# eromero-vlc/superbblas

Measured on AMD Instinct MI355X. Metric: lattice contraction GFLOP/s + permute GB/s, 16^4 spin×color, 1/2/4/8 GPUs, higher is better.
Workload: dtype complex<f64>

## Files before the change

superbblas_amd/csrc/capi.cpp:

```cpp
#include "plan.h"
#include <atomic>
#include <algorithm>
#include <functional>
#include <memory>
#include <unordered_map>

#include <rccl/rccl.h>

#include <cstdlib>
#include <cstring>
#include <mutex>

namespace sbx {
BsrOp *bsr_create(int nd, int ni, int dtype, const std::vector<std::vector<Range>> &pi,
                  const Coor &dimi, const std::vector<std::vector<Range>> &pd, const Coor &dimd,
                  const Coor &blocki, const Coor &blockd, bool block_im_fast,
                  const std::vector<const int *> &ii, const std::vector<const int *> &jj,
                  const std::vector<const void *> &v, const std::vector<int> &devs, bool reverse_jj,
                  const Comm &comm, const Coor *kroni = nullptr, const Coor *krond = nullptr,
                  const std::vector<const void *> *kronv = nullptr);
void bsr_destroy(BsrOp *op);
void bsr_krylov(const BsrOp &op, const Scalar &alpha, const std::string &oi,
                const std::string &od, const DistTensor &x, const Coor &fromx, const Coor &sizex,
                const Scalar &beta, const DistTensor &y, const Coor &fromy, const Coor &sizey,
// ... 301 lines not shown
        clear_copy_launch_cache();
        std::lock_guard<std::mutex> g(g_tape_mutex);
        tapes().clear();
    });
}

int sbx_clear_handles(void) {
    return guard([&] {
        trim_pools();
        destroy_streams();
    });
}

int sbx_allocate(unsigned long long bytes, sbx_context ctx, void **ptr) {
    return guard([&] {
        if (ctx.plat == SBX_GPU) {
            *ptr = device_alloc(bytes, ctx.device);
        } else {
            SBX_HIP_CHECK(hipHostMalloc(ptr, bytes, hipHostMallocDefault));
        }
    });
}

int sbx_deallocate(void *ptr, sbx_context ctx) {
    return guard([&] {
        if (!ptr) return;
        if (ctx.plat == SBX_GPU) {
            set_device(ctx.device);
            SBX_HIP_CHECK(hipStreamSynchronize(get_stream(ctx.device)));
            device_free(ptr, ctx.device);
        } else {
            SBX_HIP_CHECK(hipHostFree(ptr));
        }
    });
}

int sbx_set_custom_allocator(sbx_alloc_fn alloc, sbx_free_fn dealloc, void *user) {
    return guard([&] {
        if ((alloc == nullptr) != (dealloc == nullptr))
            throw Error("set_custom_allocator: give both functions or neither");
        set_alloc_hooks(alloc, dealloc, user);
    });
}

int sbx_allocate_from_cache(unsigned long long bytes, sbx_context ctx, void **ptr) {
    return guard([&] {
        if (ctx.plat != SBX_GPU) throw Error("allocate_from_cache: GPU contexts only");
        *ptr = scratch_alloc(bytes, ctx.device);
    });
}

int sbx_release_to_cache(void *ptr, sbx_context ctx) {
    return guard([&] {
        if (ctx.plat != SBX_GPU) throw Error("release_to_cache: GPU contexts only");
        scratch_free(ptr, ctx.device);
    });
}

int sbx_cache_usage(int device, unsigned long long *cached, unsigned long long *live) {
    return guard([&] {
        std::size_t c = 0, l = 0;
        cache_usage(device, &c, &l);
        if (cached) *cached = c;
        if (live) *live = l;
    });
}

int sbx_tune_set(const char *key, long long value) {
    return guard([&] {
        if (!key) throw Error("tune_set: null key");
        const std::string k(key);
        if (k == "copy.budget") g_copy_tune.budget = (long)value;
        else if (k == "copy.run") g_copy_tune.run = (long)value;
        else if (k == "copy.nt") g_copy_tune.nt = (int)value;
        else if (k == "copy.max_elems") g_copy_tune.max_elems = (long)value;
        else if (k == "copy.pair") g_copy_tune.pair = (int)value;
        else if (k == "copy.order") g_copy_tune.order = (int)value;
        else if (k == "copy.trans") g_copy_tune.trans = (int)value;
        else if (k == "copy.btrans") g_copy_tune.btrans = (int)value;
        else if (k == "gemm.max_bytes") g_gemm_tune.max_bytes = (long)value;
        else if (k == "gemm.loaders") g_gemm_tune.loaders = (int)value;
        else if (k == "gemm.dma_spread") g_gemm_tune.dma_spread = (int)value;
        else if (k == "gemm.dma_nt") g_gemm_tune.dma_nt = (int)value;
        else if (k == "gemm.skinny") g_gemm_tune.skinny = (int)value;
        else if (k == "bsr.variant") g_bsr_tune.variant = (int)value;
        else if (k == "bsr.row_max_cols") g_bsr_tune.row_max_cols = (long)value;
        else if (k == "bsr.split_max_cols") g_bsr_tune.split_max_cols = (long)value;
        else if (k == "bsr.split_cw") g_bsr_tune.split_cw = (int)value;
        else if (k == "bsr.split_jb") g_bsr_tune.split_jb = (int)value;
        else if (k == "bsr.split_ilv") g_bsr_tune.split_ilv = (int)value;
        else if (k == "bsr.kron_mfma") g_bsr_tune.kron_mfma = (int)value;
        else if (k == "bsr.kron_mfma_min_cols") g_bsr_tune.kron_mfma_min_cols = (long)value;
        else if (k == "bsr.kron_pack") g_bsr_tune.kron_pack = (int)value;
        else if (k == "bsr.kron_xlds") g_bsr_tune.kron_xlds = (int)value;
        else if (k == "bsr.kron_ylds") g_bsr_tune.kron_ylds = (int)value;
        else if (k == "bsr.kron_spin") g_bsr_tune.kron_spin = (int)value;
        else if (k == "bsr.kron_spin_min_cols") g_bsr_tune.kron_spin_min_cols = (long)value;
        else if (k == "bsr.kron_order") g_bsr_tune.kron_order = (int)value;
        else if (k == "bsr.nt") g_bsr_tune.nt = (int)value;
        else if (k == "dense.wave") g_dense_wave = (int)value;
        else if (k == "bsr.blk_pd") g_bsr_tune.blk_pd = (int)value;
        else if (k == "bsr.tile") g_bsr_tune.tile = (int)value;
        else if (k == "bsr.tile_min_cols") g_bsr_tune.tile_min_cols = value;
        else if (k == "gemm.m3") g_gemm_tune.m3 = (int)value;
        else if (k == "gemm.splits") g_gemm_tune.splits = (int)value;
        else if (k == "gemm.t48") g_gemm_tune.t48 = (int)value;
        else if (k == "gemm.share_ab") g_gemm_tune.share_ab = (int)value;
        else if (k == "gemm.herm") g_gemm_tune.herm = (int)value;
        else if (k == "gemm.frag") g_gemm_tune.frag = (int)value;
        else if (k == "gemm.dot_wgs") g_gemm_tune.dot_wgs = (int)value;
        else if (k == "gemm.frag_tall") g_gemm_tune.frag_tall = (int)value;
        else if (k == "gemm.frag_pair") g_gemm_tune.frag_pair = (int)value;
        else if (k == "gemm.frag_nt") g_gemm_tune.frag_nt = (int)value;
        else if (k == "gemm.frag_small") g_gemm_tune.frag_small = (int)value;
        else if (k == "gemm.frag_uk") g_gemm_tune.frag_uk = (int)value;
        else if (k == "gemm.frag_waves") g_gemm_tune.frag_waves = (int)value;
        else if (k == "gemm.clock") {
            g_gemm_tune.clock = (int)value;
            unsigned long long v[3];
            gemm_clock_read(current_device(), v, true);
        }
        else if (k == "dist.reduce") g_dist_reduce = (int)value;
        else if (k == "debug.level") g_debug_level = (int)value;
        else if (k == "debug.corrupt_copy") g_debug_corrupt = (int)value;
        else if (k == "dist.reduce_calls") g_dist_reduce_calls = value;
        else if (k == "dist.force_peer") g_dist_force_peer = (int)value;
        else if (k == "dist.peer_copies") g_dist_peer_copies = value;
        else if (k.compare(0, 6, "alloc.") == 0) alloc_tune(key, nullptr, &value);
        else throw Error("tune_set: unknown key " + k);
        if (k.compare(0, 5, "copy.") == 0) {
            std::lock_guard<std::mutex> g(g_tape_mutex);
            tapes().clear();
        }
    });
}

int sbx_tune_get(const char *key, long long *value) {
    return guard([&] {
        if (!key || !value) throw Error("tune_get: null argument");
        const std::string k(key);
        if (k == "copy.budget") *value = g_copy_tune.budget;
        else if (k == "copy.run") *value = g_copy_tune.run;
        else if (k == "copy.nt") *value = g_copy_tune.nt;
        else if (k == "copy.max_elems") *value = g_copy_tune.max_elems;
        else if (k == "copy.pair") *value = g_copy_tune.pair;
        else if (k == "copy.order") *value = g_copy_tune.order;
        else if (k == "copy.trans") *value = g_copy_tune.trans;
        else if (k == "copy.btrans") *value = g_copy_tune.btrans;
        else if (k == "copy.last_pair") *value = g_copy_tune.last_pair;
        else if (k == "gemm.max_bytes") *value = g_gemm_tune.max_bytes;
        else if (k == "gemm.loaders") *value = g_gemm_tune.loaders;
        else if (k == "gemm.dma_spread") *value = g_gemm_tune.dma_spread;
        else if (k == "gemm.dma_nt") *value = g_gemm_tune.dma_nt;
        else if (k == "gemm.skinny") *value = g_gemm_tune.skinny;
        else if (k == "bsr.variant") *value = g_bsr_tune.variant;
        else if (k == "bsr.row_max_cols") *value = g_bsr_tune.row_max_cols;
        else if (k == "bsr.split_max_cols") *value = g_bsr_tune.split_max_cols;
        else if (k == "bsr.split_cw") *value = g_bsr_tune.split_cw;
        else if (k == "bsr.split_jb") *value = g_bsr_tune.split_jb;
        else if (k == "bsr.split_ilv") *value = g_bsr_tune.split_ilv;
        else if (k == "bsr.kron_mfma") *value = g_bsr_tune.kron_mfma;
        else if (k == "bsr.kron_mfma_min_cols") *value = g_bsr_tune.kron_mfma_min_cols;
        else if (k == "bsr.kron_pack") *value = g_bsr_tune.kron_pack;
        else if (k == "bsr.kron_xlds") *value = g_bsr_tune.kron_xlds;
        else if (k == "bsr.kron_ylds") *value = g_bsr_tune.kron_ylds;
        else if (k == "bsr.kron_spin") *value = g_bsr_tune.kron_spin;
        else if (k == "bsr.kron_spin_min_cols") *value = g_bsr_tune.kron_spin_min_cols;
        else if (k == "bsr.kron_order") *value = g_bsr_tune.kron_order;
        else if (k == "bsr.nt") *value = g_bsr_tune.nt;
        else if (k == "dense.wave") *value = g_dense_wave;
        else if (k == "bsr.blk_pd") *value = g_bsr_tune.blk_pd;
        else if (k == "bsr.tile") *value = g_bsr_tune.tile;
        else if (k == "bsr.tile_min_cols") *value = g_bsr_tune.tile_min_cols;
        else if (k == "bsr.last_kernel") *value = g_bsr_tune.last;
        else if (k == "gemm.m3") *value = g_gemm_tune.m3;
        else if (k == "gemm.splits") *value = g_gemm_tune.splits;
        else if (k == "gemm.t48") *value = g_gemm_tune.t48;
        else if (k == "gemm.share_ab") *value = g_gemm_tune.share_ab;
        else if (k == "gemm.herm") *value = g_gemm_tune.herm;
        else if (k == "gemm.last_herm") *value = g_gemm_tune.last_herm;
        else if (k == "gemm.frag") *value = g_gemm_tune.frag;
        else if (k == "gemm.dot_wgs") *value = g_gemm_tune.dot_wgs;
        else if (k == "gemm.frag_tall") *value = g_gemm_tune.frag_tall;
        else if (k == "gemm.frag_pair") *value = g_gemm_tune.frag_pair;
        else if (k == "gemm.frag_nt") *value = g_gemm_tune.frag_nt;
        else if (k == "gemm.frag_small") *value = g_gemm_tune.frag_small;
        else if (k == "gemm.frag_uk") *value = g_gemm_tune.frag_uk;
        else if (k == "gemm.frag_waves") *value = g_gemm_tune.frag_waves;
        else if (k == "gemm.clock") *value = g_gemm_tune.clock;
        else if (k == "gemm.clock_cycles" || k == "gemm.clock_ticks" || k == "gemm.clock_launches") {
            unsigned long long v[3];
            gemm_clock_read(current_device(), v, false);
            *value = (long long)v[k == "gemm.clock_cycles" ? 0 : k == "gemm.clock_ticks" ? 1 : 2];
        }
        else if (k == "dist.reduce") *value = g_dist_reduce;
        else if (k == "debug.level") *value = g_debug_level;
        else if (k == "debug.corrupt_copy") *value = g_debug_corrupt;
        else if (k == "dist.reduce_calls") *value = g_dist_reduce_calls;
        else if (k == "dist.force_peer") *value = g_dist_force_peer;
        else if (k == "dist.peer_copies") *value = g_dist_peer_copies;
        else if (k == "detail.last_device") *value = g_detail_last_device;
        else if (k.compare(0, 6, "alloc.") == 0) alloc_tune(key, value, nullptr);
        else throw Error("tune_get: unknown key " + k);
    });
}

int sbx_timings_enable(int on) {
    return guard([&] { timings_enable(on != 0); });
}

int sbx_timings_filter(const char *names) {
    return guard([&] { timings_filter(names && *names ? names : nullptr); });
}

int sbx_timings_reset(void) {
    return guard([&] { timings_reset(); });
}

int sbx_timings_get(const char *name, double *ms, long long *calls) {
    return guard([&] {
        if (!name || !ms || !calls) throw Error("timings_get: null argument");
        timings_get(name, ms, calls);
    });
}

int sbx_timings_report(char *buf, int len) {
    return guard([&] {
        const std::string r = timings_report();
        if (buf && len > 0) {
            const int n = std::min((int)r.size(), len - 1);
            std::memcpy(buf, r.data(), n);
            buf[n] = 0;
        }
    });
}

// ... 1008 lines not shown
```

superbblas_amd/csrc/kernels_gemm.hip:

```cpp
#include "sbx_internal.h"

#include <algorithm>
#include <map>
#include <mutex>
#include <cstdint>
#include <type_traits>

namespace sbx {
GemmTune g_gemm_tune;
namespace {

template <typename R> struct Mfma;
template <> struct Mfma<double> {
    typedef double acc_t __attribute__((ext_vector_type(4)));
    static __device__ __forceinline__ acc_t mma(double a, double b, acc_t c) {
        return __builtin_amdgcn_mfma_f64_16x16x4f64(a, b, c, 0, 0, 0);
    }
    static __device__ __forceinline__ int row(int lane, int r) { return (lane >> 4) + 4 * r; }
};
template <> struct Mfma<float> {
    typedef float acc_t __attribute__((ext_vector_type(4)));
    static __device__ __forceinline__ acc_t mma(float a, float b, acc_t c) {
        return __builtin_amdgcn_mfma_f32_16x16x4f32(a, b, c, 0, 0, 0);
    }
// ... 684 lines not shown
            __syncthreads();
            if (kg == g) {
#pragma unroll
                for (int i = 0; i < MT; ++i)
#pragma unroll
                    for (int j = 0; j < NT; ++j)
#pragma unroll
                        for (int r = 0; r < 4; ++r) {
                            E v;
                            if constexpr (CPLX) v = E{accR[i][j][r], accI[i][j][r]};
                            else v = accR[i][j][r];
                            red[(((w2 * MT + i) * NT + j) * 4 + r) * 64 + lane] = v;
                        }
            }
            __syncthreads();
            if (kg == 0) {
#pragma unroll
                for (int i = 0; i < MT; ++i)
#pragma unroll
                    for (int j = 0; j < NT; ++j)
#pragma unroll
                        for (int r = 0; r < 4; ++r) {
                            const E v = red[(((w2 * MT + i) * NT + j) * 4 + r) * 64 + lane];
                            if constexpr (CPLX) {
                                accR[i][j][r] += v.x;
                                accI[i][j][r] += v.y;
                            } else {
                                accR[i][j][r] += v;
                            }
                        }
            }
        }
        if (kg != 0) return;
    }
    if (p.probe && bid == 0 && tid == 0) {
        const unsigned long long clk1 = __builtin_amdgcn_s_memtime();
        const unsigned long long rt1 = __builtin_amdgcn_s_memrealtime();
        if (p.probe_all < 0) {
            atomicAdd(&p.probe[0], clk1 - clk0);
            atomicAdd(&p.probe[1], rt1 - rt0);
            atomicAdd(&p.probe[2], 1ull);
        } else {
            p.probe[0] = clk1 - clk0;
            p.probe[1] = rt1 - rt0;
        }
    }
    if (p.probe && p.probe_all > 0 && tid == 0) {
        p.probe[2 + 3 * bid] = rt0;
        p.probe[3 + 3 * bid] = __builtin_amdgcn_s_memrealtime();
    }
    const int ccol = lane & 15;
    auto put = [&](long gi, long gj, R vr, R vi) {
        if (p.splits == 1) {
            R *cptr = (R *)((E *)p.c + bb * p.sc_b + c_off(p, gi, gj));
            epilogue_store<R>(cptr, vr, vi, p, CPLX);
        } else {
            E *w = (E *)p.work + (((long)split * p.batch + bb) * p.n + gj) * p.m + gi;
            if constexpr (CPLX)
                *w = E{vr, vi};
            else
                *w = vr;
        }
    };
#pragma unroll
    for (int i = 0; i < MT; ++i)
#pragma unroll
        for (int j = 0; j < NT; ++j)
#pragma unroll
            for (int r = 0; r < 4; ++r) {
                const long gi = m0 + wm * WTM + 16 * i + Mfma<R>::row(lane, r);
                const long gj = n0 + wn * WTN + 16 * j + ccol;
                if (gi >= p.m || gj >= p.n) continue;
                R vr = accR[i][j][r];
                R vi = CPLX ? accI[i][j][r] : R(0);
                if constexpr (G3) {
                    const R p1 = vr, p2 = vi;
                    vr = p1 - p2;
                    vi = acc3[i][j][r] - p1 - p2;
                }
                put(gi, gj, vr, vi);
                if constexpr (HERM) {
                    if (m0 != n0) put(gj, gi, vr, p.herm == 1 ? -vi : vi);
                }
            }
}

template <typename R, bool CPLX, bool AK, int BM, int BKK, int KG, int RING, bool FUSE = false,
          bool HERM = false>
__global__ void __launch_bounds__(KG * 64) gemm_wave_kernel(const GemmKArgs p, unsigned *counters) {
    typedef typename Elem<R, CPLX>::type E;
    typedef typename Mfma<R>::acc_t acc_t;
    constexpr int ES = (int)sizeof(E);
    constexpr int MT = BM / 16;
    static_assert(MT * 16 == BM && RING >= 2 && BKK % 4 == 0, "wave kernel shape");
    typedef DmaOperand<AK, BM, BKK, 64, ES> Op;
    constexpr int SLAB = BM * BKK;
    constexpr int NI = Op::NI;
    static_assert(NI * (RING - 1) <= 60, "vmcnt range");
    constexpr int RED_E = (KG / 2 > 1 ? KG / 2 : 1) * BM * BM;
    constexpr int LDS_E = KG * RING * SLAB > RED_E ? KG * RING * SLAB : RED_E;
    __shared__ __attribute__((aligned(16))) E lds[LDS_E];

    const int nwg = gridDim.x, bid = blockIdx.x;
    const int xcd = bid & 7, q = nwg >> 3, rr = nwg & 7;
    const int wg = (xcd < rr ? xcd * (q + 1) : rr * (q + 1) + (xcd - rr) * q) + (bid >> 3);
    const int split = wg % p.splits;
    const long bb = wg / p.splits;
    const long k_begin = (long)split * p.kchunk;
    const long k_end = min(p.k, k_begin + p.kchunk);
    const E *A = (const E *)p.a + bb * p.sa_b;
    const __amdgpu_buffer_rsrc_t rsA =
        __builtin_amdgcn_make_buffer_rsrc((void *)A, (short)0, (int)p.a_bytes, 0x00020000);
    const int tid = threadIdx.x, lane = tid & 63;
    const int wave = __builtin_amdgcn_readfirstlane(tid >> 6);
    const bool spl = p.split != 0;
    Op da;
    da.init(lane, 0, p.m, p.sa_m, p.sa_k, spl, p.m_lo, p.sa_m_hi);
    const long nsl = (k_end - k_begin + BKK - 1) / BKK;
    const long per = (nsl + KG - 1) / KG;
    const long s0 = min(nsl, (long)wave * per), s1 = min(nsl, s0 + per);
    const char *const mine = (const char *)lds + (size_t)wave * RING * SLAB * ES;
    auto issue = [&](long sl) {
        da.issue(rsA, mine + (size_t)((sl - s0) % RING) * SLAB * ES, 0, k_begin + sl * BKK, k_end,
                 p.sa_k, spl, p.k_lo, p.sa_k_hi);
    };
    typedef typename std::conditional<sizeof(R) == 8, unsigned long long, unsigned>::type U;
    const U sign = (U)1 << (sizeof(R) * 8 - 1);
    const U ma = p.conja ? sign : 0, mb = p.conjb ? sign : 0;
    auto flip = [](R v, U m) { return __builtin_bit_cast(R, __builtin_bit_cast(U, v) ^ m); };
    acc_t accR[MT][MT], accI[MT][MT];
#pragma unroll
    for (int i = 0; i < MT; ++i)
#pragma unroll
        for (int j = 0; j < MT; ++j) {
            accR[i][j] = acc_t{0, 0, 0, 0};
            accI[i][j] = acc_t{0, 0, 0, 0};
        }
    const int frow = lane & 15, kq = lane >> 4;
#pragma unroll
    for (int r = 0; r < RING - 1; ++r)
        if (s0 + r < s1) issue(s0 + r);
    for (long sl = s0; sl < s1; ++sl) {
        const long sn = sl + RING - 1;
        if (sn < s1) {
            asm volatile("s_waitcnt lgkmcnt(0)" ::: "memory");
            issue(sn);
        }
        const long after = min((long)(RING - 1), s1 - 1 - sl);
        if constexpr (RING >= 3) {
            if (after >= 2) asm volatile("s_waitcnt vmcnt(%0)" ::"n"(2 * NI) : "memory");
            else if (after == 1) asm volatile("s_waitcnt vmcnt(%0)" ::"n"(NI) : "memory");
            else asm volatile("s_waitcnt vmcnt(0)" ::: "memory");
        } else {
            if (after >= 1) asm volatile("s_waitcnt vmcnt(%0)" ::"n"(NI) : "memory");
            else asm volatile("s_waitcnt vmcnt(0)" ::: "memory");
        }
        const E *As = (const E *)(mine + (size_t)((sl - s0) % RING) * SLAB * ES);
#pragma unroll
        for (int kk = 0; kk < BKK; kk += 4) {
            E af[MT], bf[MT];
#pragma unroll
            for (int i = 0; i < MT; ++i) af[i] = As[Op::slot(frow + 16 * i, kk + kq)];
#pragma unroll
            for (int j = 0; j < MT; ++j) bf[j] = af[j];
            if constexpr (CPLX) {
#pragma unroll
// ... 522 lines not shown
    }
    launch_reduce<R, CPLX>(p, stream);
}

static unsigned long long *g_clock_meter[64];
static std::mutex g_clock_mu;

unsigned long long *gemm_clock_meter(int device) {
    if (g_gemm_tune.clock <= 0 || device < 0 || device >= 64) return nullptr;
    std::lock_guard<std::mutex> lock(g_clock_mu);
    if (!g_clock_meter[device]) {
        void *ptr = nullptr;
        SBX_HIP_CHECK(hipMalloc(&ptr, 3 * sizeof(unsigned long long)));
        SBX_HIP_CHECK(hipMemset(ptr, 0, 3 * sizeof(unsigned long long)));
        g_clock_meter[device] = (unsigned long long *)ptr;
    }
    return g_clock_meter[device];
}

void clock_read_impl(int device, unsigned long long out[3], bool reset) {
    out[0] = out[1] = out[2] = 0;
    std::lock_guard<std::mutex> lock(g_clock_mu);
    if (device < 0 || device >= 64 || !g_clock_meter[device]) return;
    SBX_HIP_CHECK(hipDeviceSynchronize());
    SBX_HIP_CHECK(hipMemcpy(out, g_clock_meter[device], 3 * sizeof(unsigned long long),
                            hipMemcpyDeviceToHost));
    if (reset) SBX_HIP_CHECK(hipMemset(g_clock_meter[device], 0, 3 * sizeof(unsigned long long)));
}

template <typename R, bool CPLX, bool AK, bool BK, int BM, int BN, int BKK, int WM, int WN,
          bool ALLOW_M3 = true, bool PF = false, int KG = 1, bool SH = false, int LW = 0, int SP = 1,
          bool HERM_OK = false>
void launch_dma_cfg(const GemmKArgs &p0, int device, hipStream_t stream, long splits = 0,
                    long target_wgs = 1024) {
    const bool m3 = CPLX && g_gemm_tune.m3 > 0;
    GemmKArgs p = p0;
    Scratch work;
    if (g_gemm_tune.splits > 0) splits = g_gemm_tune.splits;
    p.dma_nt = g_gemm_tune.dma_nt;
    p.same_ab = g_gemm_tune.share_ab && same_operands(p);
    long nwg = prepare_launch<typename Elem<R, CPLX>::type>(p, BM, BN, BKK, splits, target_wgs,
                                                            work, device);
    if (SH && !(p.same_ab && p.tm == 1 && p.tn == 1))
        throw Error("gemm: internal error, shared slab image for a launch with off-diagonal tiles");
    static_assert(!HERM_OK || (AK == BK && BM == BN && !PF && KG == 1 && !SH), "Hermitian output");
    if constexpr (HERM_OK) {
        if (!m3 && p.tm > 1) p.herm = herm_mode<typename Elem<R, CPLX>::type>(p, CPLX);
        if (p.herm) {
            nwg = (long)p.tm * (p.tm + 1) / 2 * p.batch * p.splits;
            g_gemm_tune.last_herm = p.tm * (p.tm - 1) / 2;
        }
    }
    if (unsigned long long *meter = gemm_clock_meter(device)) {
        p.probe = meter;
        p.probe_all = -1;
    }
    KernelTimer total("gemm_total", stream);
    {
        KernelTimer timer("gemm", stream);
        bool launched = false;
        if constexpr (HERM_OK) {
            if (p.herm) {
                hipLaunchKernelGGL((gemm_dma_kernel<R, CPLX, AK, BK, BM, BN, BKK, WM, WN, false, PF, KG, SH, LW, SP, true>),
                                   dim3((unsigned)nwg), dim3(WM * WN * KG * 64), 0, stream, p);
                launched = true;
            }
        }
        if (launched) {
        } else if constexpr (ALLOW_M3) {
            if (m3)
                hipLaunchKernelGGL((gemm_dma_kernel<R, CPLX, AK, BK, BM, BN, BKK, WM, WN, CPLX>),
                                   dim3((unsigned)nwg), dim3(WM * WN * 64), 0, stream, p);
            else
                hipLaunchKernelGGL((gemm_dma_kernel<R, CPLX, AK, BK, BM, BN, BKK, WM, WN>),
                                   dim3((unsigned)nwg), dim3(WM * WN * 64), 0, stream, p);
        } else
            hipLaunchKernelGGL((gemm_dma_kernel<R, CPLX, AK, BK, BM, BN, BKK, WM, WN, false, PF, KG, SH, LW, SP>),
                               dim3((unsigned)nwg), dim3(WM * WN * KG * 64), 0, stream, p);
        SBX_HIP_CHECK(hipGetLastError());
    }
    launch_reduce<R, CPLX>(p, stream);
}

unsigned *splitk_counters(hipStream_t stream, long n, int device) {
    static std::mutex mu;
    static std::map<hipStream_t, std::pair<unsigned *, long>> arrays;
    std::lock_guard<std::mutex> lock(mu);
    auto &a = arrays[stream];
    if (a.second < n) {
        if (a.first) {
            SBX_HIP_CHECK(hipStreamSynchronize(stream));
            SBX_HIP_CHECK(hipFree(a.first));
        }
        const long cap = std::max(n, 1024L);
        void *ptr = nullptr;
        SBX_HIP_CHECK(hipMalloc(&ptr, sizeof(unsigned) * cap));
        SBX_HIP_CHECK(hipMemset(ptr, 0, sizeof(unsigned) * cap));
        a = {(unsigned *)ptr, cap};
    }
    (void)device;
    return a.first;
}

template <typename R, bool CPLX, bool AK, int BM, int BKK, int KG, int RING, bool FUSE = false>
void launch_wave_cfg(const GemmKArgs &p0, int device, hipStream_t stream, long target_wgs) {
    GemmKArgs p = p0;
    Scratch work;
    long splits = g_gemm_tune.splits > 0 ? g_gemm_tune.splits : 0;
    const long nwg = prepare_launch<typename Elem<R, CPLX>::type>(p, BM, BM, BKK * KG, splits,
                                                                   target_wgs, work, device);
    if (p.tm != 1 || p.tn != 1 || p.m != p.n)
        throw Error("gemm: internal error, wave kernel for a launch with several tiles");
    unsigned *counters = FUSE && p.splits > 1 ? splitk_counters(stream, p.batch, device) : nullptr;
    constexpr int MT = BM / 16;
    p.herm = MT > 1 ? herm_mode<typename Elem<R, CPLX>::type>(p, CPLX) : 0;
    if (p.herm) g_gemm_tune.last_herm = MT * (MT - 1) / 2;
    KernelTimer total("gemm_total", stream);
    {
        KernelTimer timer("gemm", stream);
        if (p.herm)
            hipLaunchKernelGGL((gemm_wave_kernel<R, CPLX, AK, BM, BKK, KG, RING, FUSE, true>),
                               dim3((unsigned)nwg), dim3(KG * 64), 0, stream, p, counters);
        else
            hipLaunchKernelGGL((gemm_wave_kernel<R, CPLX, AK, BM, BKK, KG, RING, FUSE>),
                               dim3((unsigned)nwg), dim3(KG * 64), 0, stream, p, counters);
        SBX_HIP_CHECK(hipGetLastError());
    }
    if (!FUSE) launch_reduce<R, CPLX>(p, stream);
}

template <typename E> bool dma_ok(const GemmKArgs &p, bool ak, bool bk) {
    constexpr long EPG = 16 / (long)sizeof(E);
    if (EPG == 1) return true;
    auto aligned = [](const void *ptr) { return ((std::uintptr_t)ptr & 15) == 0; };
    if (!aligned(p.a) || !aligned(p.b)) return false;
    if (p.split) {
        if ((ak ? p.k_lo : p.m_lo) % EPG || (bk ? p.k_lo : p.n_lo) % EPG) return false;
        if (p.sa_m_hi % EPG || p.sa_k_hi % EPG || p.sb_k_hi % EPG || p.sb_n_hi % EPG) return false;
    }
    if (ak && (p.k % EPG || p.sa_m % EPG || p.sa_b % EPG)) return false;
    if (bk && (p.k % EPG || p.sb_n % EPG || p.sb_b % EPG)) return false;
    if (!ak && (p.m % EPG || p.sa_k % EPG || p.sa_b % EPG)) return false;
    if (!bk && (p.n % EPG || p.sb_k % EPG || p.sb_b % EPG)) return false;
    return true;
}

template <typename R, bool CPLX, bool AK, bool BK>
void launch_tiled(const GemmKArgs &p, int device, hipStream_t stream) {
    typedef typename Elem<R, CPLX>::type E;
    constexpr bool HM = AK == BK;
    if (!dma_ok<E>(p, AK, BK)) {
        launch_tiled_cfg<R, CPLX, AK, BK, 64, 64, 16, 2, 2>(p, device, stream);
    } else if constexpr (std::is_same<R, double>::value && CPLX) {
        const bool m3 = g_gemm_tune.m3 > 0;
        if (p.m >= 128 && p.n >= 128) {
            if (m3)
                launch_dma_cfg<R, CPLX, AK, BK, 128, 128, 8, 4, 2>(p, device, stream, 0, 256);
            else if constexpr (AK && BK) {
                const int lw = p.split ? 0 : g_gemm_tune.loaders, sp = g_gemm_tune.dma_spread;
                if (lw == 4 && sp == 4)
                    launch_dma_cfg<R, CPLX, AK, BK, 128, 128, 16, 4, 4, false, false, 1, false, 4, 4>(p, device, stream, 0, 256);
                else if (lw == 4)
                    launch_dma_cfg<R, CPLX, AK, BK, 128, 128, 16, 4, 4, false, false, 1, false, 4, 1>(p, device, stream, 0, 256);
                else if (lw == 8 && sp == 4)
                    launch_dma_cfg<R, CPLX, AK, BK, 128, 128, 16, 4, 4, false, false, 1, false, 8, 4>(p, device, stream, 0, 256);
                else if (lw == 8 && sp == 0)
                    launch_dma_cfg<R, CPLX, AK, BK, 128, 128, 16, 4, 4, false, false, 1, false, 8, 0>(p, device, stream, 0, 256);
                else if (lw == 8)
                    launch_dma_cfg<R, CPLX, AK, BK, 128, 128, 16, 4, 4, false, false, 1, false, 8, 1, true>(p, device, stream, 0, 256);
                else if (lw == 16 && sp == 4)
                    launch_dma_cfg<R, CPLX, AK, BK, 128, 128, 16, 4, 4, false, false, 1, false, 16, 4>(p, device, stream, 0, 256);
                else
                    launch_dma_cfg<R, CPLX, AK, BK, 128, 128, 16, 4, 4, false, false, 1, false, 0, 1, HM>(p, device, stream, 0, 256);
            } else
                launch_dma_cfg<R, CPLX, AK, BK, 128, 128, 16, 4, 4, false, false, 1, false, 0, 1, HM>(p, device, stream, 0, 256);
        } else {
            launch_dma_cfg<R, CPLX, AK, BK, 64, 64, 8, 2, 2, true, false, 1, false, 0, 1, HM>(p, device, stream, 0, 1024);
        }
    } else {
        const int t48 = g_gemm_tune.t48;
        if (t48 > 0 && p.m > 32 && p.m <= 48 && p.n > 32 && p.n <= 48) {
            if (t48 == 1) return launch_dma_cfg<R, CPLX, AK, BK, 48, 48, 16, 3, 1>(p, device, stream, 0, 1024);
            if (t48 == 2) return launch_dma_cfg<R, CPLX, AK, BK, 48, 48, 16, 1, 3>(p, device, stream, 0, 1024);
            if (t48 == 3) return launch_dma_cfg<R, CPLX, AK, BK, 48, 48, 32, 3, 1>(p, device, stream, 0, 1024);
            if (t48 == 4) return launch_dma_cfg<R, CPLX, AK, BK, 48, 48, 16, 3, 1>(p, device, stream, 0, 1536);
            const bool sh = g_gemm_tune.share_ab && same_operands(p);
            if constexpr (!AK && !BK && sizeof(E) >= 8) {
                if (sh && t48 == 13) return launch_wave_cfg<R, CPLX, AK, 48, 8, 4, 2>(p, device, stream, 1024);
                if (sh && t48 == 14) return launch_wave_cfg<R, CPLX, AK, 48, 16, 4, 2>(p, device, stream, 768);
                if (sh && t48 == 16) return launch_wave_cfg<R, CPLX, AK, 48, 8, 16, 2>(p, device, stream, 256);
                if (sh && t48 == 17) return launch_wave_cfg<R, CPLX, AK, 48, 8, 8, 2, true>(p, device, stream, 512);
                if (sh && t48 != 6) return launch_wave_cfg<R, CPLX, AK, 48, 8, 8, 2>(p, device, stream, 512);
            }
            return launch_dma_cfg<R, CPLX, AK, BK, 48, 48, 32, 1, 1, false, false, 4>(p, device, stream, 0, 768);
        }
        if (p.m >= 128 && p.n >= 128)
            launch_dma_cfg<R, CPLX, AK, BK, 128, 128, 32, 4, 2, true, false, 1, false, 0, 1, HM>(p, device, stream, 0, 256);
        else
            launch_dma_cfg<R, CPLX, AK, BK, 64, 64, 32, 2, 2, true, false, 1, false, 0, 1, HM>(p, device, stream, 0, 1024);
    }
}

template <typename R, bool CPLX> bool launch_skinny(const GemmKArgs &p0, int device, hipStream_t s) {
    if (!g_gemm_tune.skinny || p0.split) return false;
    typedef typename Elem<R, CPLX>::type E;
    GemmKArgs p = p0;
    if (p.m <= 4 && p.n <= 4) {
        const long wgs = std::max(1, g_gemm_tune.dot_wgs);
        long splits = std::max(1L, std::min((wgs + p.batch - 1) / p.batch, (p.k + 1023) / 1024));
        p.kchunk = (p.k + splits - 1) / splits;
        splits = std::max(1L, (p.k + p.kchunk - 1) / p.kchunk);
        p.splits = (int)splits;
        Scratch work;
        if (splits > 1) {
            work = Scratch(sizeof(E) * splits * p.batch * p.m * p.n, device);
            p.work = work.ptr;
        }
        const long nwg = p.batch * splits;
        if (nwg > 0x7fffffffL) return false;
        KernelTimer total("gemm_total", s);
        {
            KernelTimer timer("gemm", s);
            const long mx = std::max(p.m, p.n);
            if (mx == 1)
                hipLaunchKernelGGL((gemm_dot_kernel<R, CPLX, 1, 1>), dim3((unsigned)nwg), dim3(256), 0, s, p);
            else if (mx == 2)
                hipLaunchKernelGGL((gemm_dot_kernel<R, CPLX, 2, 2>), dim3((unsigned)nwg), dim3(256), 0, s, p);
            else
                hipLaunchKernelGGL((gemm_dot_kernel<R, CPLX, 4, 4>), dim3((unsigned)nwg), dim3(256), 0, s, p);
            SBX_HIP_CHECK(hipGetLastError());
        }
        launch_reduce<R, CPLX>(p, s);
        return true;
    }
    const bool rows = p.n <= 16 && p.m >= 2 * p.n && p.k <= 64;
    const bool cols = p.m <= 16 && p.n >= 2 * p.m && p.k <= 64;
    if (!rows && !cols) return false;
    if (!rows) {
        std::swap(p.m, p.n);
        std::swap(p.a, p.b);
        std::swap(p.sa_m, p.sb_n);
        std::swap(p.sa_k, p.sb_k);
        std::swap(p.sa_b, p.sb_b);
// ... 151 lines not shown

}

void gemm_clock_read(int device, unsigned long long out[3], bool reset) {
    clock_read_impl(device, out, reset);
}

void launch_gemm(const GemmDesc &d, int device) {
    if (d.m == 0 || d.n == 0 || d.batch == 0) return;
    if (d.k > 0 && (d.alpha.re != 0 || d.alpha.im != 0)) {
        const long es = (long)dtype_size(d.t);
        const long max_bytes = g_gemm_tune.max_bytes > 0 ? g_gemm_tune.max_bytes : (1L << 31) - 1;
        auto ext = [&](long n, long lo, long st, long st_hi) {
            return lo > 0 && lo < n ? (n / lo - 1) * std::labs(st_hi) + (lo - 1) * std::labs(st)
                                    : (n - 1) * std::labs(st);
        };
        const long ea = (ext(d.m, d.m_lo, d.sa_m, d.sa_m_hi) + ext(d.k, d.k_lo, d.sa_k, d.sa_k_hi) + 1) * es;
        const long eb = (ext(d.k, d.k_lo, d.sb_k, d.sb_k_hi) + ext(d.n, d.n_lo, d.sb_n, d.sb_n_hi) + 1) * es;
        if (ea > max_bytes || eb > max_bytes) {
            struct Cut {
                long n1, lo1, n2, lo2, o_outer;
                bool ok;
            };
            auto cut = [](long n, long lo) {
                Cut c{};
                const bool spl = lo > 0 && lo < n;
                if (spl) {
                    const long outer = n / lo, o1 = outer / 2;
                    c = Cut{o1 * lo, lo, n - o1 * lo, lo, o1, true};
                } else {
                    c = Cut{n / 2, 0, n - n / 2, 0, n / 2, n > 1};
                }
                return c;
            };
            auto off = [](long n, long lo, long st, long st_hi, long o) {
                return lo > 0 && lo < n ? o * st_hi : o * st;
            };
            const Cut ck = cut(d.k, d.k_lo);
            if (ck.ok) {
                GemmDesc a = d, b = d;
                a.k = ck.n1;
                a.k_lo = ck.lo1;
                b.k = ck.n2;
                b.k_lo = ck.lo2;
                b.a = (const char *)d.a + es * off(d.k, d.k_lo, d.sa_k, d.sa_k_hi, ck.o_outer);
                b.b = (const char *)d.b + es * off(d.k, d.k_lo, d.sb_k, d.sb_k_hi, ck.o_outer);
                b.beta = Scalar{1, 0};
                launch_gemm(a, device);
                launch_gemm(b, device);
                return;
            }
            const Cut cm = cut(d.m, d.m_lo), cn = cut(d.n, d.n_lo);
            if (cm.ok && (ea > max_bytes || !cn.ok)) {
                GemmDesc a = d, b = d;
                a.m = cm.n1;
                a.m_lo = cm.lo1;
                b.m = cm.n2;
                b.m_lo = cm.lo2;
                b.a = (const char *)d.a + es * off(d.m, d.m_lo, d.sa_m, d.sa_m_hi, cm.o_outer);
                b.c = (char *)d.c + es * off(d.m, d.m_lo, d.sc_m, d.sc_m_hi, cm.o_outer);
                launch_gemm(a, device);
                launch_gemm(b, device);
                return;
            }
            if (cn.ok) {
                GemmDesc a = d, b = d;
                a.n = cn.n1;
                a.n_lo = cn.lo1;
                b.n = cn.n2;
                b.n_lo = cn.lo2;
                b.b = (const char *)d.b + es * off(d.n, d.n_lo, d.sb_n, d.sb_n_hi, cn.o_outer);
                b.c = (char *)d.c + es * off(d.n, d.n_lo, d.sc_n, d.sc_n_hi, cn.o_outer);
                launch_gemm(a, device);
                launch_gemm(b, device);
                return;
            }
            throw Error("gemm: operand batch entries of 2 GiB or more are not supported");
        }
    }
    set_device(device);
    hipStream_t s = get_stream(device);
    GemmKArgs p = make_args(d);
    g_gemm_tune.last_herm = 0;
    const bool scale_only = (d.k == 0 || (p.alpha_re == 0 && p.alpha_im == 0));
    switch (d.t) {
    case SBX_CDOUBLE:
        scale_only ? launch_scale<double, true>(p, s) : launch_typed<double, true>(p, device, s);
        break;
    case SBX_DOUBLE:
        scale_only ? launch_scale<double, false>(p, s) : launch_typed<double, false>(p, device, s);
        break;
    case SBX_CFLOAT:
        scale_only ? launch_scale<float, true>(p, s) : launch_typed<float, true>(p, device, s);
        break;
    case SBX_FLOAT:
        scale_only ? launch_scale<float, false>(p, s) : launch_typed<float, false>(p, device, s);
        break;
    default: throw Error("gemm: unsupported type");
    }
}

}
```

superbblas_amd/csrc/sbx_internal.h:

```cpp
#pragma once

#include <hip/hip_runtime.h>

#include <array>
#include <atomic>
#include <complex>
#include <cstdint>
#include <cstring>
#include <memory>
#include <stdexcept>
#include <string>
#include <vector>

#include "../../include/superbblas_amd/sbx.h"

namespace sbx {

struct Error : public std::runtime_error {
    explicit Error(const std::string &s) : std::runtime_error(s) {}
};

#define SBX_HIP_CHECK(expr)                                                                        \
    do {                                                                                           \
        hipError_t sbx_e_ = (expr);                                                                \
// ... 71 lines not shown
void timings_get(const char *name, double *ms, long long *calls);
std::string timings_report();
void timings_filter(const char *names);
struct KernelTimer {
    const char *name;
    hipStream_t stream;
    void *ev0 = nullptr;
    KernelTimer(const char *name, hipStream_t s);
    ~KernelTimer();
};


struct GemmDesc {
    int t;
    long m, n, k, batch;
    const void *a;
    long sa_m, sa_k, sa_b;
    bool conja;
    const void *b;
    long sb_k, sb_n, sb_b;
    bool conjb;
    void *c;
    long sc_m, sc_n, sc_b;
    Scalar alpha, beta;
    long m_lo = 0, n_lo = 0, k_lo = 0;
    long sa_m_hi = 0, sa_k_hi = 0, sb_k_hi = 0, sb_n_hi = 0, sc_m_hi = 0, sc_n_hi = 0;
};
void launch_gemm(const GemmDesc &d, int device);

struct BoxCopyDesc {
    int src_t, dst_t;
    const void *src;
    void *dst;
    std::vector<long> size, src_stride, dst_stride;
    Scalar alpha;
    bool add;
    const float *src_mask = nullptr, *dst_mask = nullptr;
};
void launch_box_copy(const BoxCopyDesc &d, int device);
void clear_copy_launch_cache();
int copy_kernel_plan(const BoxCopyDesc &d, long *blocks);

struct TapeLaunch {
    std::shared_ptr<const void> launch;
    const void *src;
    void *dst;
    int device;
    Scalar alpha;
    int src_arg = -1, src_comp = -1, dst_arg = -1, dst_comp = -1;
    long src_off = 0, dst_off = 0;
    bool alpha_is_call = false;
};
struct CopyTape {
    std::vector<TapeLaunch> launches;
    bool valid = true;
};
void set_copy_tape(CopyTape *t);
CopyTape *current_copy_tape();
void replay_launch(const TapeLaunch &l, const void *src, void *dst, const Scalar &alpha);
void clear_copy_plan_cache();
struct CopyTune {
    long budget = 0;
    long run = 0;
    int nt = 0;
    long max_elems = 0;
    int pair = 0;
    int order = 0;
    int trans = 0;
    int btrans = 0;
    std::atomic<int> last_pair{0};
};
extern CopyTune g_copy_tune;
struct GemmTune {
    int m3 = 0;
    int splits = 0;
    long max_bytes = 0;
    int t48 = 5;
    int share_ab = 1;
    int herm = 0;
    std::atomic<int> last_herm{0};
    int loaders = 8;
    int dma_spread = 1;
    int dma_nt = 0;
    int skinny = 1;
    int clock = 0;
    int dot_wgs = 256;
    int frag_uk = 0;
    int frag_waves = 4096;
    int frag = 1;
    int frag_small = 32;
    int frag_nt = 0;
    int frag_pair = 1;
    int frag_tall = 0;
};
uint32_t storage_checksum(const void *p, std::size_t bytes, std::size_t blocksize, uint32_t prev);
void gemm_clock_read(int device, unsigned long long out[3], bool reset);
extern GemmTune g_gemm_tune;
struct BsrTune {
    int variant = 0;
    long row_max_cols = 3;
    long split_max_cols = 32;
    int split_cw = 0;
    int split_jb = 0;
    int split_ilv = 2;
    int kron_mfma = 1;
    long kron_mfma_min_cols = 8;
    int kron_pack = 1;
    int kron_xlds = 1;
    int kron_ylds = 0;
    int kron_spin = 0;
    long kron_spin_min_cols = 8;
    int kron_order = 1;
    int blk_pd = 1;
    int tile = 0;
    long tile_min_cols = 33;
    int nt = 11;
    std::atomic<int> last{0};
};
extern BsrTune g_bsr_tune;
extern int g_dense_wave;

inline void check_dma_lds(const char *kernel, size_t lds, long passes, long lanes_per_pass,
                   long extra_bytes = 0) {
    const long need = passes * lanes_per_pass * 16 + extra_bytes;
    if ((long)lds < need)
        throw Error(std::string("bsr: internal LDS sizing error in ") + kernel + ": " +
                    std::to_string(lds) + " bytes for DMA passes needing " + std::to_string(need));
}

void launch_zero(void *p, std::size_t bytes, int device);

struct IndexCopyDesc {
    int src_t, dst_t;
    const void *src;
    void *dst;
    const int *src_idx = nullptr, *dst_idx = nullptr;
    long n = 0, blocking = 1;
    Scalar alpha;
    bool add = false;
};
void launch_index_copy(const IndexCopyDesc &d, int device);

struct TileSched {
    const int *rows = nullptr, *uniq = nullptr;
    const unsigned char *loc = nullptr;
    int umax = 0, tt = 0;
    long chunks = 0;
};

struct BsrDesc {
    int t;
    long block_rows;
    int bi, bd;
    const int *ii;
    const int *jj;
    const void *v;
    bool block_im_fast;
    int num_nnz_per_row;
    const void *x;
    long ldx;
    long x_rows = 0;
    bool x_row_major;
    void *y;
    long ldy;
    bool y_row_major;
    long ncols;
// ... 27 lines not shown
```

Before: 69730.

## Add lean complex-f64 MFMA GEMM kernel with LDS-direct double-buffered DMA

Adds a specialized complex-double GEMM kernel for 128x128 tiles that loads A and B directly into LDS using buffer_load with the lds modifier, double-buffered across 16-wide K slabs. Conjugation is folded into the MFMA negate modifiers, so each conjugation combination gets its own template instance. The kernel is enabled by default whenever the dimensions divide the tile sizes and the default loader configuration is in use. The aim is lower per-slab address and instruction overhead than the generic DMA configuration, at the cost of a narrow, hand-scheduled path that relies on inline asm and the m0 register.

```diff
diff --git a/superbblas_amd/csrc/capi.cpp b/superbblas_amd/csrc/capi.cpp
--- a/superbblas_amd/csrc/capi.cpp
+++ b/superbblas_amd/csrc/capi.cpp
@@ -407,6 +407,7 @@
         else if (k == "gemm.loaders") g_gemm_tune.loaders = (int)value;
         else if (k == "gemm.dma_spread") g_gemm_tune.dma_spread = (int)value;
         else if (k == "gemm.dma_nt") g_gemm_tune.dma_nt = (int)value;
+        else if (k == "gemm.lean") g_gemm_tune.lean = (int)value;
         else if (k == "gemm.skinny") g_gemm_tune.skinny = (int)value;
         else if (k == "bsr.variant") g_bsr_tune.variant = (int)value;
         else if (k == "bsr.row_max_cols") g_bsr_tune.row_max_cols = (long)value;
@@ -477,6 +478,8 @@
         else if (k == "gemm.loaders") *value = g_gemm_tune.loaders;
         else if (k == "gemm.dma_spread") *value = g_gemm_tune.dma_spread;
         else if (k == "gemm.dma_nt") *value = g_gemm_tune.dma_nt;
+        else if (k == "gemm.lean") *value = g_gemm_tune.lean;
+        else if (k == "gemm.last_lean") *value = g_gemm_tune.last_lean;
         else if (k == "gemm.skinny") *value = g_gemm_tune.skinny;
         else if (k == "bsr.variant") *value = g_bsr_tune.variant;
         else if (k == "bsr.row_max_cols") *value = g_bsr_tune.row_max_cols;
diff --git a/superbblas_amd/csrc/kernels_gemm.hip b/superbblas_amd/csrc/kernels_gemm.hip
--- a/superbblas_amd/csrc/kernels_gemm.hip
+++ b/superbblas_amd/csrc/kernels_gemm.hip
@@ -790,6 +790,189 @@
                 if constexpr (HERM) {
                     if (m0 != n0) put(gj, gi, vr, p.herm == 1 ? -vi : vi);
                 }
+            }
+}
+
+template <int NEG>
+__device__ __forceinline__ Mfma<double>::acc_t mma_f64(double a, double b, Mfma<double>::acc_t c) {
+    return __builtin_amdgcn_mfma_f64_16x16x4f64(a, b, c, 0, 0, NEG);
+}
+
+template <int OFF>
+__device__ __forceinline__ void lean_dma_piece(unsigned voff, unsigned sbase,
+                                               __amdgpu_buffer_rsrc_t rs, unsigned soff) {
+    asm volatile("s_add_u32 m0, %1, %4\n\t"
+                 "s_nop 0\n\t"
+                 "buffer_load_dwordx4 %0, %2, %3 offen lds"
+                 :
+                 : "v"(voff), "s"(sbase), "s"(rs), "s"(soff), "n"(OFF)
+                 : "memory", "m0", "scc");
+}
+
+template <bool CA, bool CB>
+__global__ void __launch_bounds__(1024) gemm_lean_kernel(const GemmKArgs p) {
+    typedef double R;
+    typedef double2 E;
+    typedef Mfma<R>::acc_t acc_t;
+    constexpr int BM = 128, BN = 128, BKK = 16, WN = 4, WTM = 32, WTN = 32, MT = 2, NT = 2;
+    constexpr int ES = 16, LW = 8, NI = 4, RSTEP = 32;
+    constexpr int SLAB = (BM + BN) * BKK;
+    constexpr unsigned IMG_B = BM * BKK * ES, SLAB_B = SLAB * ES, PIECE_B = LW * 64 * 16;
+    typedef DmaOperand<true, BM, BKK, 1024, ES> Op;
+    __shared__ __attribute__((aligned(16))) E lds[2 * SLAB];
+
+    const int nwg = gridDim.x, bid = blockIdx.x;
+    const int xcd = bid & 7, q = nwg >> 3, rr = nwg & 7;
+    const int wg = (xcd < rr ? xcd * (q + 1) : rr * (q + 1) + (xcd - rr) * q) + (bid >> 3);
+    const int ti = wg % p.tm;
+    int rest = wg / p.tm;
+    const int tj = rest % p.tn;
+    rest /= p.tn;
+    const int split = rest % p.splits;
+    const long bb = rest / p.splits;
+    const long m0 = (long)ti * BM, n0 = (long)tj * BN;
+    const long k_begin = (long)split * p.kchunk;
+    const long k_end = min(p.k, k_begin + p.kchunk);
+
+    const E *A = (const E *)p.a + bb * p.sa_b;
+    const E *B = (const E *)p.b + bb * p.sb_b;
+    const __amdgpu_buffer_rsrc_t rsA =
+        __builtin_amdgcn_make_buffer_rsrc((void *)A, (short)0, (int)p.a_bytes, 0x00020000);
+    const __amdgpu_buffer_rsrc_t rsB =
+        __builtin_amdgcn_make_buffer_rsrc((void *)B, (short)0, (int)p.b_bytes, 0x00020000);
+
+    const int tid = threadIdx.x, lane = tid & 63;
+    const int wave = __builtin_amdgcn_readfirstlane(tid >> 6);
+    unsigned long long clk0 = 0, rt0 = 0;
+    if (p.probe && bid == 0) {
+        clk0 = __builtin_amdgcn_s_memtime();
+        rt0 = __builtin_amdgcn_s_memrealtime();
+    }
+    const bool loader = wave < LW;
+    unsigned va[NI], vb[NI];
+    {
+        const int r = tid >> 4, k = (tid & 15) ^ (r & 15);
+#pragma unroll
+        for (int i = 0; i < NI; ++i) {
+            va[i] = (unsigned)(((m0 + r + RSTEP * i) * p.sa_m + (long)k * p.sa_k) * ES);
+            vb[i] = (unsigned)(((n0 + r + RSTEP * i) * p.sb_n + (long)k * p.sb_k) * ES);
+        }
+    }
+    unsigned ka = (unsigned)(k_begin * p.sa_k * ES), kb = (unsigned)(k_begin * p.sb_k * ES);
+    const unsigned ka_step = (unsigned)(BKK * p.sa_k * ES), kb_step = (unsigned)(BKK * p.sb_k * ES);
+    const unsigned lbase = lds_addr(lds) + (unsigned)wave * (64 * 16);
+    auto issue = [&](unsigned sb) {
+        lean_dma_piece<0 * PIECE_B>(va[0], sb, rsA, ka);
+        lean_dma_piece<1 * PIECE_B>(va[1], sb, rsA, ka);
+        lean_dma_piece<2 * PIECE_B>(va[2], sb, rsA, ka);
+        lean_dma_piece<3 * PIECE_B>(va[3], sb, rsA, ka);
+        lean_dma_piece<IMG_B + 0 * PIECE_B>(vb[0], sb, rsB, kb);
+        lean_dma_piece<IMG_B + 1 * PIECE_B>(vb[1], sb, rsB, kb);
+        lean_dma_piece<IMG_B + 2 * PIECE_B>(vb[2], sb, rsB, kb);
+        lean_dma_piece<IMG_B + 3 * PIECE_B>(vb[3], sb, rsB, kb);
+    };
+
+    const int wm = wave / WN, wn = wave % WN;
+    const int frow = wm * WTM + (lane & 15), fcol = wn * WTN + (lane & 15), kq = lane >> 4;
+    int fa[BKK / 4], fb[BKK / 4];
+#pragma unroll
+    for (int s = 0; s < BKK / 4; ++s) {
+        fa[s] = Op::slot(frow, 4 * s + kq);
+        fb[s] = BM * BKK + Op::slot(fcol, 4 * s + kq);
+    }
+
+    acc_t accR[MT][NT], accI[MT][NT];
+#pragma unroll
+    for (int i = 0; i < MT; ++i)
+#pragma unroll
+        for (int j = 0; j < NT; ++j) {
+            accR[i][j] = acc_t{0, 0, 0, 0};
+            accI[i][j] = acc_t{0, 0, 0, 0};
+        }
+
+    const int nslab = (int)((k_end - k_begin) / BKK);
+    if (nslab > 0 && loader) issue(lbase);
+    for (int s = 0; s < nslab; ++s) {
+        asm volatile("s_waitcnt vmcnt(0)" ::: "memory");
+        __syncthreads();
+        const int cur = s & 1;
+        ka += ka_step;
+        kb += kb_step;
+        if (loader && s + 1 < nslab) issue(lbase + (unsigned)(cur ^ 1) * SLAB_B);
+        const E *L = lds + cur * SLAB;
+#pragma unroll
+        for (int ks = 0; ks < BKK / 4; ++ks) {
+            E af[MT], bf[NT];
+#pragma unroll
+            for (int i = 0; i < MT; ++i) af[i] = L[fa[ks] + 16 * i * BKK];
+#pragma unroll
+            for (int j = 0; j < NT; ++j) bf[j] = L[fb[ks] + 16 * j * BKK];
+#pragma unroll
+            for (int i = 0; i < MT; ++i)
+#pragma unroll
+                for (int j = 0; j < NT; ++j) {
+                    accR[i][j] = mma_f64<0>(af[i].x, bf[j].x, accR[i][j]);
+                    accI[i][j] = mma_f64<CB ? 1 : 0>(af[i].x, bf[j].y, accI[i][j]);
+                }
+#pragma unroll
+            for (int i = 0; i < MT; ++i)
+#pragma unroll
+                for (int j = 0; j < NT; ++j) {
+                    accR[i][j] = mma_f64<CA == CB ? 1 : 0>(af[i].y, bf[j].y, accR[i][j]);
+                    accI[i][j] = mma_f64<CA ? 1 : 0>(af[i].y, bf[j].x, accI[i][j]);
+                }
+        }
+    }
+
+    if (p.probe && bid == 0 && tid == 0) {
+        const unsigned long long clk1 = __builtin_amdgcn_s_memtime();
+        const unsigned long long rt1 = __builtin_amdgcn_s_memrealtime();
+        if (p.probe_all < 0) {
+            atomicAdd(&p.probe[0], clk1 - clk0);
+            atomicAdd(&p.probe[1], rt1 - rt0);
+            atomicAdd(&p.probe[2], 1ull);
+        } else {
+            p.probe[0] = clk1 - clk0;
+            p.probe[1] = rt1 - rt0;
+        }
+    }
+    const int ccol = lane & 15;
+    if (p.splits > 1) {
+        E *const w0 = (E *)p.work + (((long)split * p.batch + bb) * p.n + n0) * p.m + m0;
+#pragma unroll
+        for (int half = 0; half < 2; ++half) {
+            __syncthreads();
+            if ((wn >> 1) == half) {
+#pragma unroll
+                for (int i = 0; i < MT; ++i)
+#pragma unroll
+                    for (int j = 0; j < NT; ++j)
+#pragma unroll
+                        for (int r = 0; r < 4; ++r) {
+                            const int row = wm * WTM + 16 * i + Mfma<R>::row(lane, r);
+                            const int col = (wn & 1) * WTN + 16 * j + ccol;
+                            lds[col * BM + (row ^ (col & 7))] = E{accR[i][j][r], accI[i][j][r]};
+                        }
+            }
+            __syncthreads();
+#pragma unroll
+            for (int pass = 0; pass < 64 * BM / 1024; ++pass) {
+                const int idx = pass * 1024 + tid, col = idx / BM, row = idx % BM;
+                w0[(long)(half * 64 + col) * p.m + row] = lds[col * BM + (row ^ (col & 7))];
+            }
+        }
+        return;
+    }
+#pragma unroll
+    for (int i = 0; i < MT; ++i)
+#pragma unroll
+        for (int j = 0; j < NT; ++j)
+#pragma unroll
+            for (int r = 0; r < 4; ++r) {
+                const long gi = m0 + wm * WTM + 16 * i + Mfma<R>::row(lane, r);
+                const long gj = n0 + wn * WTN + 16 * j + ccol;
+                R *cptr = (R *)((E *)p.c + bb * p.sc_b + gi * p.sc_m + gj * p.sc_n);
+                epilogue_store<R>(cptr, accR[i][j][r], accI[i][j][r], p, true);
             }
 }
 
@@ -1478,6 +1661,40 @@
     launch_reduce<R, CPLX>(p, stream);
 }
 
+bool lean_eligible(const GemmKArgs &p) {
+    if (!g_gemm_tune.lean || g_gemm_tune.m3 > 0 || g_gemm_tune.dma_nt || p.split) return false;
+    if (p.m % 128 || p.n % 128 || p.k % 16) return false;
+    if ((g_gemm_tune.share_ab || g_gemm_tune.herm) && same_operands(p)) return false;
+    return !(p.probe && p.probe_all > 0);
+}
+
+void launch_lean(const GemmKArgs &p0, int device, hipStream_t stream) {
+    GemmKArgs p = p0;
+    Scratch work;
+    const long nwg = prepare_launch<double2>(p, 128, 128, 16, g_gemm_tune.splits > 0 ? g_gemm_tune.splits : 0,
+                                             256, work, device);
+    if (unsigned long long *meter = gemm_clock_meter(device)) {
+        p.probe = meter;
+        p.probe_all = -1;
+    }
+    g_gemm_tune.last_lean = 1;
+    KernelTimer total("gemm_total", stream);
+    {
+        KernelTimer timer("gemm", stream);
+        const dim3 grid((unsigned)nwg), block(1024);
+        if (p.conja && p.conjb)
+            hipLaunchKernelGGL((gemm_lean_kernel<true, true>), grid, block, 0, stream, p);
+        else if (p.conja)
+            hipLaunchKernelGGL((gemm_lean_kernel<true, false>), grid, block, 0, stream, p);
+        else if (p.conjb)
+            hipLaunchKernelGGL((gemm_lean_kernel<false, true>), grid, block, 0, stream, p);
+        else
+            hipLaunchKernelGGL((gemm_lean_kernel<false, false>), grid, block, 0, stream, p);
+        SBX_HIP_CHECK(hipGetLastError());
+    }
+    launch_reduce<double, true>(p, stream);
+}
+
 unsigned *splitk_counters(hipStream_t stream, long n, int device) {
     static std::mutex mu;
     static std::map<hipStream_t, std::pair<unsigned *, long>> arrays;
@@ -1554,7 +1771,9 @@
                 launch_dma_cfg<R, CPLX, AK, BK, 128, 128, 8, 4, 2>(p, device, stream, 0, 256);
             else if constexpr (AK && BK) {
                 const int lw = p.split ? 0 : g_gemm_tune.loaders, sp = g_gemm_tune.dma_spread;
-                if (lw == 4 && sp == 4)
+                if (lw == 8 && sp == 1 && lean_eligible(p))
+                    launch_lean(p, device, stream);
+                else if (lw == 4 && sp == 4)
                     launch_dma_cfg<R, CPLX, AK, BK, 128, 128, 16, 4, 4, false, false, 1, false, 4, 4>(p, device, stream, 0, 256);
                 else if (lw == 4)
                     launch_dma_cfg<R, CPLX, AK, BK, 128, 128, 16, 4, 4, false, false, 1, false, 4, 1>(p, device, stream, 0, 256);
@@ -1872,6 +2091,7 @@
     hipStream_t s = get_stream(device);
     GemmKArgs p = make_args(d);
     g_gemm_tune.last_herm = 0;
+    g_gemm_tune.last_lean = 0;
     const bool scale_only = (d.k == 0 || (p.alpha_re == 0 && p.alpha_im == 0));
     switch (d.t) {
     case SBX_CDOUBLE:
diff --git a/superbblas_amd/csrc/sbx_internal.h b/superbblas_amd/csrc/sbx_internal.h
--- a/superbblas_amd/csrc/sbx_internal.h
+++ b/superbblas_amd/csrc/sbx_internal.h
@@ -177,6 +177,8 @@
     int loaders = 8;
     int dma_spread = 1;
     int dma_nt = 0;
+    int lean = 1;
+    std::atomic<int> last_lean{0};
     int skinny = 1;
     int clock = 0;
     int dot_wgs = 256;
```

Result: faster. 73760 (median of 6 runs) (+5.8%).
